# avlmaps/AVLMaps

Measured on AMD Instinct MI355X. Metric: voxel_query_similarities_per_sec, higher is better.
Workload: dtype f32

## Files before the change

avlmaps_amd/_lib.py:

```python
from __future__ import annotations

import ctypes as C
import os
import sys
import threading
from pathlib import Path

_PKG = Path(__file__).resolve().parent
LIB_PATH = Path(os.environ.get("AVLMAPS_HIP_LIB") or _PKG / "lib" / "libavlmaps_hip.so")

AVL_OK = 0
SIM_AUTO, SIM_EXACT, SIM_SPLIT_F16, SIM_EXACT_VALU, SIM_PREPARED, SIM_PREPARED24 = 0, 1, 2, 3, 4, 5


class AvlError(RuntimeError):
    pass


_lib = None

_vp, _i32, _i64, _f64, _sz = C.c_void_p, C.c_int32, C.c_int64, C.c_double, C.c_size_t
_SIGS = {
    "avl_last_error": (C.c_char_p, []),
    "avl_version": (C.c_int, []),
# ... 68 lines not shown
    "avl_builder_destroy": (C.c_int, [_vp]),
    "avl_builder_reset": (C.c_int, [_vp, _vp]),
    "avl_builder_enable_replay_log": (C.c_int, [_vp, _i64]),
    "avl_builder_integrate_frame": (C.c_int, [_vp, _vp, C.c_int, C.c_int, _vp, _vp, _vp, _vp, C.c_int, _vp, C.c_int,
                                              C.c_int, _vp, _i64, _f64, _f64, _f64, _vp]),
    "avl_builder_integrate_batch": (C.c_int, [_vp, C.c_int, _vp, C.c_int, C.c_int, _vp, _vp, _vp, _vp, C.c_int, _vp, C.c_int, C.c_int,
                                              _vp, _i64, _f64, _f64, _f64, _vp]),
    "avl_builder_integrate_frames": (C.c_int, [_vp, C.c_int, _vp, C.c_int, C.c_int, _vp, _vp, _vp, _vp, C.c_int, _vp, C.c_int, C.c_int,
                                               _vp, _i64, _f64, _f64, _f64, _vp]),
    "avl_builder_integrate_frame_global": (C.c_int, [_vp, _vp, C.c_int, _f64, C.c_int, C.c_int, _vp, _vp, _vp, _vp, C.c_int, _vp,
                                                     C.c_int, C.c_int, _vp, _i64, _f64, _f64, _f64, _vp, _vp]),
    "avl_points_bbox": (C.c_int, [_vp, C.c_int, _f64, C.c_int, C.c_int, _vp, _vp, _vp, C.c_int, _f64, _f64, _vp, _vp]),
    "avl_builder_import_map": (C.c_int, [_vp, _i64, _vp, _vp, _vp, _vp, _vp]),
    "avl_builder_num_voxels": (C.c_int, [_vp, C.POINTER(_i64), _vp]),
    "avl_builder_num_points": (C.c_int, [_vp, C.POINTER(_i64), _vp]),
    "avl_builder_num_groups": (C.c_int, [_vp, C.POINTER(_i64), _vp]),
    "avl_builder_finalize": (C.c_int, [_vp, _i64, _vp, _vp, _vp, _vp, _vp, _vp]),
    "avl_builder_finalize_ex": (C.c_int, [_vp, _i64, _vp, _vp, _vp, _vp, _vp, _vp, C.c_int, _vp]),
    "avl_builder_export_raw": (C.c_int, [_vp, _i64, _vp, _vp, _vp, _vp, _vp, _vp, _vp]),
    "avl_finalize_raw": (C.c_int, [_i64, C.c_int, C.c_int, C.c_int, _vp, _vp, _vp, _vp, _vp, _vp, _vp, _vp, _vp, _vp, _vp]),
    "avl_builder_set_max_capacity": (C.c_int, [_vp, _i64]),
    "avl_builder_capacity": (C.c_int, [_vp, C.POINTER(_i64)]),
    "avl_builder_set_deferred_fuse": (C.c_int, [_vp, C.c_int, _vp]),
    "avl_builder_flush": (C.c_int, [_vp, _vp]),
    "avl_builder_release_scratch": (C.c_int, [_vp, _i64, _vp]),
    "avl_builder_scatter_merge": (C.c_int, [_vp, _i64, _vp, _vp, _vp, _i64, _vp]),
    "avl_finalize_merged": (C.c_int, [_i64, _i64, C.c_int, C.c_int, C.c_int, _vp, _vp, _i64, _vp, _vp, _vp, _vp, _vp, _vp]),
    "avl_builder_replay_chain": (C.c_int, [_vp, _i64, _vp, C.c_uint64, _vp, _vp]),
    "avl_builder_drop_replay_cache": (C.c_int, [_vp, _vp]),
    "avl_builder_replay_prepare": (C.c_int, [_vp, _i64, _vp]),
    "avl_replay_state_apply": (C.c_int, [_i64, _vp, _vp, _vp, _vp]),
    "avl_rows_add_f64": (C.c_int, [_i64, C.c_int, _vp, _i64, _i64, _vp, _i64, _vp, _i64, _vp]),
    "avl_rows_add_f64_async": (C.c_int, [_i64, C.c_int, _vp, _i64, _i64, _vp, _i64, _vp, _i64, _vp, _vp]),
    "avl_builder_export_rows_f32": (C.c_int, [_vp, _i64, _vp, _vp, _i64, _vp]),
    "avl_builder_export_rows_f64": (C.c_int, [_vp, _i64, _vp, _vp, _vp, _i64, _vp]),
    "avl_finalize_side": (C.c_int, [_i64, _i64, C.c_int, C.c_int, _vp, _vp, _vp, _vp, _vp, _vp, _vp]),
    "avl_pool_label_2d": (C.c_int, [_vp, _vp, _i64, C.c_int, _vp, _vp]),
    "avl_rgb_topdown": (C.c_int, [_vp, _vp, _i64, C.c_int, _vp, _vp]),
    "avl_obstacle_map": (C.c_int, [_vp, C.c_int, C.c_int, C.c_int, C.c_int, C.c_int, _vp, _vp]),
    "avl_obstacle_scatter": (C.c_int, [_vp, _vp, _i64, _vp, C.c_int, C.c_int, C.c_int, C.c_int, C.c_int, _vp, _vp, _vp]),
    "avl_heatmap_from_mask": (C.c_int, [_vp, _vp, _i64, _f64, _f64, _vp, _vp]),
    "avl_heat_plan_create": (C.c_int, [C.POINTER(_vp), _vp, _i64, _vp]),
    "avl_heat_plan_destroy": (C.c_int, [_vp]),
    "avl_heatmap_from_mask_planned": (C.c_int, [_vp, _vp, _f64, _f64, _vp, _vp]),
    "avl_lseg_merge_windows": (C.c_int, [_vp, C.c_int, C.c_int, C.c_int, C.c_int, _vp, C.c_int, C.c_int, _vp, _vp]),
    "avl_field_area": (C.c_int, [_vp, _vp, _i64, C.c_int, _f64, _vp, _vp, _vp]),
# ... 72 lines not shown
```

avlmaps_amd/csrc/avl_builder.hip:

```cpp
#include <algorithm>
#include <climits>
#include <cstring>
#include <vector>

#include <rocprim/device/device_radix_sort.hpp>
#include <rocprim/device/device_select.hpp>
#include <rocprim/iterator/counting_iterator.hpp>

#include "avl_common.h"

namespace avl {

#ifdef AVL_PROBE_CHAIN
__device__ unsigned long long* g_probe = nullptr;
constexpr int kProbeK12Row0 = 16384;
#define AVL_STAMP(var)                                                                                             \
    unsigned long long var;                                                                                        \
    asm volatile("s_waitcnt vmcnt(0) lgkmcnt(0)\n\ts_memrealtime %0\n\ts_waitcnt lgkmcnt(0)" : "=s"(var)::"memory")
#define AVL_STAMP_DECL(var) unsigned long long var = 0
#define AVL_RESTAMP(var) asm volatile("s_waitcnt vmcnt(0) lgkmcnt(0)\n\ts_memrealtime %0\n\ts_waitcnt lgkmcnt(0)" : "=s"(var)::"memory")
#else
#define AVL_STAMP(var)
#define AVL_STAMP_DECL(var)
#define AVL_RESTAMP(var)
// ... 75 lines not shown
    const auto p = __builtin_amdgcn_kernarg_segment_ptr();
    int t0, t1, t2, t3;
    if constexpr (LINES == 4)
        asm volatile("s_load_dword %0, %4, 0x0\n s_load_dword %1, %4, 0x40\n s_load_dword %2, %4, 0x80\n s_load_dword %3, %4, 0xc0\n"
                     "s_waitcnt lgkmcnt(0)" : "=&s"(t0), "=&s"(t1), "=&s"(t2), "=&s"(t3) : "s"(p));
    if constexpr (LINES == 8)
        asm volatile("s_load_dword %0, %4, 0x0\n s_load_dword %1, %4, 0x40\n s_load_dword %2, %4, 0x80\n s_load_dword %3, %4, 0xc0\n"
                     "s_load_dword %0, %4, 0x100\n s_load_dword %1, %4, 0x140\n s_load_dword %2, %4, 0x180\n s_load_dword %3, %4, 0x1c0\n"
                     "s_waitcnt lgkmcnt(0)" : "=&s"(t0), "=&s"(t1), "=&s"(t2), "=&s"(t3) : "s"(p));
    if constexpr (LINES == 12)
        asm volatile("s_load_dword %0, %4, 0x0\n s_load_dword %1, %4, 0x40\n s_load_dword %2, %4, 0x80\n s_load_dword %3, %4, 0xc0\n"
                     "s_load_dword %0, %4, 0x100\n s_load_dword %1, %4, 0x140\n s_load_dword %2, %4, 0x180\n s_load_dword %3, %4, 0x1c0\n"
                     "s_load_dword %0, %4, 0x200\n s_load_dword %1, %4, 0x240\n s_load_dword %2, %4, 0x280\n s_load_dword %3, %4, 0x2c0\n"
                     "s_waitcnt lgkmcnt(0)" : "=&s"(t0), "=&s"(t1), "=&s"(t2), "=&s"(t3) : "s"(p));
    if constexpr (LINES == 16)
        asm volatile("s_load_dword %0, %4, 0x0\n s_load_dword %1, %4, 0x40\n s_load_dword %2, %4, 0x80\n s_load_dword %3, %4, 0xc0\n"
                     "s_load_dword %0, %4, 0x100\n s_load_dword %1, %4, 0x140\n s_load_dword %2, %4, 0x180\n s_load_dword %3, %4, 0x1c0\n"
                     "s_load_dword %0, %4, 0x200\n s_load_dword %1, %4, 0x240\n s_load_dword %2, %4, 0x280\n s_load_dword %3, %4, 0x2c0\n"
                     "s_load_dword %0, %4, 0x300\n s_load_dword %1, %4, 0x340\n s_load_dword %2, %4, 0x380\n s_load_dword %3, %4, 0x3c0\n"
                     "s_waitcnt lgkmcnt(0)" : "=&s"(t0), "=&s"(t1), "=&s"(t2), "=&s"(t3) : "s"(p));
    (void)t0; (void)t1; (void)t2; (void)t3;
    __builtin_amdgcn_sched_barrier(0);
#endif
}

__device__ __forceinline__ int py_int(double v) {
    return (int)fmin(fmax(v, -2.0e9), 2.0e9);
}

__device__ __forceinline__ double gemv3(const double* a, double x0, double x1, double x2) {
    return fma(a[2], x2, fma(a[0], x0, a[1] * x1));
}

struct SampleRec {
    double alpha;
    int32_t cell, fpix;
    uint32_t rgbv;
    int32_t slot;
};

template <int THREADS, int MODE = 0>
__device__ __forceinline__ SampleRec bp_voxelize_body(int blk, const FrameParams& fp, const float* depth,
                                                      const int32_t* __restrict__ sample_idx, const uint8_t* rgb,
                                                      int32_t* __restrict__ cell_slot, int32_t* __restrict__ slot_cell, const Recs& recs,
                                                      unsigned long long* __restrict__ counters, int* __restrict__ err_flags,
                                                      PreRec* __restrict__ pre_out = nullptr) {
// ... 271 lines not shown
    warm_kernel_arguments<12>();
    const SampleRec r = bp_voxelize_body<256>(blockIdx.x, fp, depth, sample_idx, rgb, cell_slot, slot_cell, recs, counters, err_flags);
    link_body<true, 256>(blockIdx.x, fp.P, cell_slot, head, recs, counters, log, log_base, frame_key, fp.batch, fp.P_frame, r, err_flags, ol);
}

__global__ __launch_bounds__(256) void voxelize_link_next_kernel(FrameParams fp, const float* depth, const int32_t* __restrict__ sample_idx,
                                                                 const uint8_t* rgb, int32_t* __restrict__ cell_slot,
                                                                 int32_t* __restrict__ slot_cell, Recs recs, int32_t* __restrict__ head,
                                                                 unsigned long long* __restrict__ counters, int* __restrict__ err_flags,
                                                                 ReplayLog log, long long log_base, unsigned long long frame_key,
                                                                 FrameParams fpn, PreGather next, int gb) {
    if ((int)blockIdx.x < gb) {
        bp_voxelize_body<256, 2>((int)blockIdx.x, fpn, next.depth, next.samples, next.rgb, cell_slot, slot_cell, recs, counters, err_flags, next.out);
        return;
    }
    const int blk = (int)blockIdx.x - gb;
    warm_kernel_arguments<12>();
    SampleRec r;
    if (fp.pre) r = bp_voxelize_body<256, 1>(blk, fp, depth, sample_idx, rgb, cell_slot, slot_cell, recs, counters, err_flags);
    else r = bp_voxelize_body<256, 0>(blk, fp, depth, sample_idx, rgb, cell_slot, slot_cell, recs, counters, err_flags);
    link_body<false, 256>(blk, fp.P, cell_slot, head, recs, counters, log, log_base, frame_key, nullptr, fp.P_frame, r, err_flags);
}

template <int CH, bool FULL>
__device__ __forceinline__ void fuse_group_impl(int s0, int32_t slot, double alpha0, int32_t fpix0, uint32_t rgb0, int P, int D_rt, unsigned long long frame_key, const BatchEntry* __restrict__ batch,
                                                int P_frame, const Recs& recs, int32_t* __restrict__ head, const float* __restrict__ feat,
                                                double* __restrict__ sum_feat, double* __restrict__ sum_w4,
                                                float* __restrict__ first_feat, double* __restrict__ first_alpha,
                                                unsigned long long* __restrict__ slot_key, uint8_t* __restrict__ dirty) {
    const int D = FULL ? 256 * CH : D_rt;
    const int lane = threadIdx.x & 63;
    AVL_STAMP(pt0);
    AVL_STAMP(pt1);
    const bool is_new = slot_key[slot] == kNoKey;
    const int h0 = head[slot];
    double* sf = sum_feat + (size_t)slot * D;
    AVL_STAMP(pt2);
#ifdef AVL_PROBE_CHAIN
    int probe_n = 1;
    unsigned long long pt3 = 0, pt4 = 0;
#endif

    double acc[CH][4], old[CH][4];
    float f1[CH][4];
#pragma unroll
    for (int c = 0; c < CH; ++c)
#pragma unroll
        for (int e = 0; e < 4; ++e) { acc[c][e] = 0.0; f1[c][e] = 0.f; old[c][e] = 0.0; }
    double w4 = 0.0, a1 = 0.0, w4_old = 0.0;
    int min_s = INT_MAX;
    if (!is_new) {
#pragma unroll
        for (int c = 0; c < CH; ++c) {
            const int d = c * 256 + lane * 4;
            if (FULL || (d + 3 < D && (D & 1) == 0)) {
                const double2 q0 = *reinterpret_cast<const double2*>(sf + d), q1 = *reinterpret_cast<const double2*>(sf + d + 2);
                old[c][0] = q0.x; old[c][1] = q0.y; old[c][2] = q1.x; old[c][3] = q1.y;
            } else {
#pragma unroll
                for (int e = 0; e < 4; ++e)
                    if (d + e < D) old[c][e] = sf[d + e];
            }
        }
    }
    if (lane < 4) w4_old = is_new ? 0.0 : sum_w4[(size_t)slot * 4 + lane];

    auto row_of = [&](int cur, int32_t fpix) { return (batch ? batch[cur / P_frame].feat : feat) + (size_t)fpix * D; };
    auto load_row = [&](float (&v)[CH][4], const float* f) {
#pragma unroll
        for (int c = 0; c < CH; ++c) {
            const int d = c * 256 + lane * 4;
            if (FULL || (d + 3 < D && (D & 3) == 0)) {
                const float4 q = *reinterpret_cast<const float4*>(f + d);
// ... 23 lines not shown
        }
        if (lane < 4) w4 += lane == 0 ? alpha : alpha * (double)((rgbv >> (8 * (lane - 1))) & 0xffu);
    };
    const float* feat0 = row_of(s0, fpix0);
#ifdef AVL_ABL_K3_SINGLE
    if (true) {
#else
    if (h0 == s0) {
#endif
        float v[CH][4];
        load_row(v, feat0);
        add(s0, alpha0, rgb0, v);
#ifdef AVL_PROBE_CHAIN
        { AVL_STAMP(ptx); pt3 = pt4 = ptx; }
#endif
    } else {
        int my = lane == 0 ? s0 : INT_MAX;
        int n = 1, cur = h0;
        while (cur != s0 && n < 64 && (unsigned)cur < (unsigned)P) {
            if (lane == n) my = cur;
            ++n;
            cur = recs.next[cur];
        }
#ifdef AVL_PROBE_CHAIN
        { AVL_STAMP(ptx); pt3 = ptx; probe_n = n; }
#endif
        double a_l = 0.0;
        int32_t fp_l = 0;
        uint32_t rgb_l = 0;
        if (lane < n) {
            a_l = recs.alpha[my];
            fp_l = recs.fpix[my];
            rgb_l = recs.rgb[my];
        }
#ifdef AVL_PROBE_CHAIN
        { AVL_STAMP(ptx); pt4 = ptx; }
#endif
        int rank = 0;
        for (int j = 0; j < n; ++j) rank += __builtin_amdgcn_readlane(my, j) < my ? 1 : 0;
        const int a_lo = __double2loint(a_l), a_hi = __double2hiint(a_l);
#ifndef AVL_K3_MR
#define AVL_K3_MR 2
#endif
        constexpr int MR = CH <= 4 ? AVL_K3_MR : 1;
        for (int k0 = 0; k0 < n; k0 += MR) {
            float v[MR][CH][4];
            int cj[MR], lj[MR];
#pragma unroll
            for (int j = 0; j < MR; ++j) {
                const unsigned long long m = __ballot(lane < n && rank == k0 + j);
                lj[j] = m ? __builtin_amdgcn_readfirstlane(__ffsll((long long)m) - 1) : 0;
                cj[j] = m ? __builtin_amdgcn_readlane(my, lj[j]) : -1;
                load_row(v[j], cj[j] >= 0 ? row_of(cj[j], __builtin_amdgcn_readlane(fp_l, lj[j])) : feat0);
            }
#pragma unroll
            for (int j = 0; j < MR; ++j) {
                if (cj[j] >= 0) {
                    const double al = __hiloint2double(__builtin_amdgcn_readlane(a_hi, lj[j]), __builtin_amdgcn_readlane(a_lo, lj[j]));
                    add(cj[j], al, (uint32_t)__builtin_amdgcn_readlane((int)rgb_l, lj[j]), v[j]);
                }
            }
        }
        for (int steps = 0; cur != s0 && (unsigned)cur < (unsigned)P && steps < P; ++steps) {
            const int nxt = recs.next[cur];
            float v[CH][4];
            load_row(v, row_of(cur, recs.fpix[cur]));
            add(cur, recs.alpha[cur], recs.rgb[cur], v);
            cur = nxt;
        }
    }

    AVL_STAMP(pt5);
    float* ff = first_feat + (size_t)slot * D;
#pragma unroll
    for (int c = 0; c < CH; ++c) {
        const int d = c * 256 + lane * 4;
        double r[4];
#pragma unroll
        for (int e = 0; e < 4; ++e) r[e] = is_new ? acc[c][e] : old[c][e] + acc[c][e];
        if constexpr (FULL) {
            *reinterpret_cast<double2*>(sf + d) = double2{r[0], r[1]};
            *reinterpret_cast<double2*>(sf + d + 2) = double2{r[2], r[3]};
            if (is_new) *reinterpret_cast<float4*>(ff + d) = float4{f1[c][0], f1[c][1], f1[c][2], f1[c][3]};
        } else {
#pragma unroll
            for (int e = 0; e < 4; ++e)
                if (d + e < D) {
                    sf[d + e] = r[e];
                    if (is_new) ff[d + e] = f1[c][e];
                }
        }
    }
    if (lane < 4) sum_w4[(size_t)slot * 4 + lane] = w4_old + w4;
    if (is_new) {
        if (lane == 0) {
            first_alpha[slot] = a1;
            slot_key[slot] = batch ? (batch[min_s / P_frame].frame_key | (unsigned)(min_s % P_frame)) : (frame_key | (unsigned)min_s);
        }
    }
    if (lane == 0) {
        head[slot] = -1;
        dirty[slot] = 1;
    }
#ifdef AVL_PROBE_CHAIN
    {
        AVL_STAMP(pt6);
        if (g_probe && lane == 0 && P < kProbeK12Row0) {
            unsigned long long* q = g_probe + (size_t)s0 * 8;
            q[0] = pt0; q[1] = pt1; q[2] = pt2; q[3] = pt3; q[4] = pt4; q[5] = pt5; q[6] = pt6;
            q[7] = (unsigned long long)probe_n | (is_new ? 1ull << 32 : 0ull);
        }
    }
#endif
}

template <int CH, bool COMPACT = false>
__device__ __forceinline__ void fuse_body(int blk, int P, int D, unsigned long long frame_key, const BatchEntry* __restrict__ batch,
                                          int P_frame, const Recs& recs, int32_t* __restrict__ head, const float* __restrict__ feat,
                                          double* __restrict__ sum_feat, double* __restrict__ sum_w4,
                                          float* __restrict__ first_feat, double* __restrict__ first_alpha,
                                          unsigned long long* __restrict__ slot_key, uint8_t* __restrict__ dirty,
                                          const OwnerList& ol = OwnerList{}) {
    auto group = [&](int s0, int32_t slot, double alpha0, int32_t fpix0, uint32_t rgb0) {
        if (D == 256 * CH)
            fuse_group_impl<CH, true>(s0, slot, alpha0, fpix0, rgb0, P, D, frame_key, batch, P_frame, recs, head, feat, sum_feat, sum_w4, first_feat,
                                      first_alpha, slot_key, dirty);
        else
            fuse_group_impl<CH, false>(s0, slot, alpha0, fpix0, rgb0, P, D, frame_key, batch, P_frame, recs, head, feat, sum_feat, sum_w4, first_feat,
                                       first_alpha, slot_key, dirty);
    };
    if constexpr (!COMPACT) {
        const int s0 = __builtin_amdgcn_readfirstlane((int)((blk * AVL_K3_THREADS + threadIdx.x) >> 6));
        if (s0 >= P) return;
        const uint8_t own = recs.owner[s0];
        const int32_t slot = recs.slot[s0];
        const double alpha0 = recs.alpha[s0];
        const int32_t fpix0 = recs.fpix[s0];
        const uint32_t rgb0 = recs.rgb[s0];
        if (!own) return;
        group(s0, slot, alpha0, fpix0, rgb0);
        return;
    } else {
    const int nb = (P + 255) / 256;
    const int nblk = nb * (kFuseWaves / 4);
    const int t = (int)(threadIdx.x >> 6) * nblk + blk;
    const int b = __builtin_amdgcn_readfirstlane(t / kFuseWaves);
    if (b >= nb) return;
    const int n_own = __builtin_amdgcn_readfirstlane(ol.ocnt[b]);
    for (int k = t % kFuseWaves; k < n_own; k += kFuseWaves) {
        const int oi = __builtin_amdgcn_readfirstlane(b * 256 + k);
        const double a0 = ol.o_alpha[oi];
        group(__builtin_amdgcn_readfirstlane(ol.o_s[oi]), __builtin_amdgcn_readfirstlane(ol.o_slot[oi]),
              __hiloint2double(__builtin_amdgcn_readfirstlane(__double2hiint(a0)), __builtin_amdgcn_readfirstlane(__double2loint(a0))),
              __builtin_amdgcn_readfirstlane(ol.o_fpix[oi]), (uint32_t)__builtin_amdgcn_readfirstlane((int)ol.o_rgb[oi]));
    }
    }
}

#ifndef AVL_K3_WPE
#define AVL_K3_WPE 0
#endif
#if AVL_K3_WPE
#define AVL_K3_OCC(CH) __attribute__((amdgpu_waves_per_eu((CH) <= 2 ? AVL_K3_WPE : 1)))
#else
#define AVL_K3_OCC(CH)
#endif

template <int CH, bool COMPACT>
__global__ __launch_bounds__(COMPACT ? 256 : AVL_K3_THREADS) AVL_K3_OCC(CH) void fuse_kernel(int P, int D, unsigned long long frame_key, const BatchEntry* __restrict__ batch,
                                                   int P_frame, Recs recs, int32_t* __restrict__ head, const float* __restrict__ feat,
                                                   double* __restrict__ sum_feat, double* __restrict__ sum_w4,
                                                   float* __restrict__ first_feat, double* __restrict__ first_alpha,
                                                   unsigned long long* __restrict__ slot_key, uint8_t* __restrict__ dirty, OwnerList ol) {
    fuse_body<CH, COMPACT>(blockIdx.x, P, D, frame_key, batch, P_frame, recs, head, feat, sum_feat, sum_w4, first_feat, first_alpha, slot_key, dirty, ol);
}

struct FusePrev {
    int P;
    unsigned long long frame_key;
    Recs recs;
    int32_t* head;
    const float* feat;
};

template <int CH>
__global__ __launch_bounds__(AVL_K3_THREADS) AVL_K3_OCC(CH) void pipe_kernel(FrameParams fp, int pb, const float* depth, const int32_t* __restrict__ sample_idx,
                                                   const uint8_t* rgb, int32_t* __restrict__ cell_slot, int32_t* __restrict__ slot_cell,
                                                   Recs recs, int32_t* __restrict__ head, unsigned long long* __restrict__ counters,
                                                   int* __restrict__ err_flags, ReplayLog log, long long log_base,
                                                   unsigned long long frame_key, FusePrev prev, int D, double* __restrict__ sum_feat,
                                                   double* __restrict__ sum_w4, float* __restrict__ first_feat,
                                                   double* __restrict__ first_alpha, unsigned long long* __restrict__ slot_key,
                                                   uint8_t* __restrict__ dirty, FrameParams fpn, PreGather next, int gb) {
    if ((int)blockIdx.x < gb) {
        bp_voxelize_body<AVL_K3_THREADS, 2>((int)blockIdx.x, fpn, next.depth, next.samples, next.rgb, cell_slot, slot_cell, recs, counters, err_flags,
                                            next.out);
        return;
// ... 7 lines not shown
        link_body<false, AVL_K3_THREADS>(blk, fp.P, cell_slot, head, recs, counters, log, log_base, frame_key, nullptr, fp.P_frame, r, err_flags);
    } else {
        fuse_body<CH>(blk - pb, prev.P, D, prev.frame_key, nullptr, prev.P, prev.recs, prev.head, prev.feat, sum_feat, sum_w4,
                      first_feat, first_alpha, slot_key, dirty);
    }
}

constexpr int kGenTile = 8;
__global__ __launch_bounds__(256) void fuse_generic_kernel(int P, int D, unsigned long long frame_key,
                                                           const BatchEntry* __restrict__ batch, int P_frame, Recs recs,
                                                           int32_t* __restrict__ head, const float* __restrict__ feat,
                                                           double* __restrict__ sum_feat, double* __restrict__ sum_w4,
                                                           float* __restrict__ first_feat, double* __restrict__ first_alpha,
                                                           unsigned long long* __restrict__ slot_key, uint8_t* __restrict__ dirty) {
    __shared__ int ord_s[4][64];
    const int lane = threadIdx.x & 63;
    int* ord = ord_s[(threadIdx.x >> 6) & 3];
    const int s0 = (blockIdx.x * blockDim.x + threadIdx.x) >> 6;
    if (s0 >= P) return;
    if (!recs.owner[s0]) return;
    const int32_t slot = recs.slot[s0];
    const bool is_new = slot_key[slot] == kNoKey;
    const int h0 = head[slot];
    auto wave_max = [&](int v) {
#pragma unroll
        for (int o = 32; o >= 1; o >>= 1) v = max(v, __shfl_xor(v, o));
        return v;
    };
    int n_total = 0, min_s = INT_MAX, held = INT_MAX;
    for (int cur = h0; cur >= 0 && (unsigned)cur < (unsigned)P && n_total < P; cur = recs.next[cur]) {
        if (n_total < 64 && lane == n_total) held = cur;
        min_s = min(min_s, cur);
        ++n_total;
    }
    if (n_total == 0) return;
    const double a1 = recs.alpha[min_s];
    const float* row1 = (batch ? batch[min_s / P_frame].feat : feat) + (size_t)recs.fpix[min_s] * D;
    double* sf = sum_feat + (size_t)slot * D;
    float* ff = first_feat + (size_t)slot * D;
    if (is_new)
        for (int d = lane; d < D; d += 64) ff[d] = row1[d];
    double w4 = 0.0;
    int prev = -1;
    bool first_round = true;
    for (int done = 0; done < n_total;) {
        int m;
        if (n_total <= 64) {
            m = n_total;
        } else {
            held = INT_MAX;
            int cnt = 0, curmax = -1, steps = 0;
            for (int cur = h0; cur >= 0 && (unsigned)cur < (unsigned)P && steps < P; cur = recs.next[cur], ++steps) {
                if (cur <= prev) continue;
                if (cnt < 64) {
                    if (lane == cnt) held = cur;
                    if (++cnt == 64) curmax = wave_max(held);
                } else if (cur < curmax) {
                    const unsigned long long at = __ballot(held == curmax);
                    if (lane == __ffsll((long long)at) - 1) held = cur;
                    curmax = wave_max(held);
                }
            }
            m = cnt;
            if (m == 0) break;
        }
        int rank = 0;
        for (int j = 0; j < m; ++j) rank += __builtin_amdgcn_readlane(held, j) < held ? 1 : 0;
        if (lane < m) ord[rank] = held;
        __builtin_amdgcn_wave_barrier();
        prev = ord[m - 1];
        for (int k = 0; k < m; ++k) {
            const int cur = ord[k];
            const double alpha = recs.alpha[cur];
            const uint32_t rgbv = recs.rgb[cur];
            if (lane < 4) w4 += lane == 0 ? alpha : alpha * (double)((rgbv >> (8 * (lane - 1))) & 0xffu);
        }
        for (int d0 = 0; d0 < D; d0 += 64 * kGenTile) {
            double acc[kGenTile];
#pragma unroll
            for (int t = 0; t < kGenTile; ++t) acc[t] = 0.0;
            for (int k = 0; k < m; ++k) {
                const int cur = ord[k];
                if (is_new && cur == min_s) continue;
                const double alpha = recs.alpha[cur];
                const float* row = (batch ? batch[cur / P_frame].feat : feat) + (size_t)recs.fpix[cur] * D;
#pragma unroll
                for (int t = 0; t < kGenTile; ++t) {
                    const int d = d0 + t * 64 + lane;
                    if (d < D) acc[t] += alpha * (double)row[d];
                }
            }
#pragma unroll
            for (int t = 0; t < kGenTile; ++t) {
                const int d = d0 + t * 64 + lane;
                if (d < D) sf[d] = (is_new && first_round) ? acc[t] : sf[d] + acc[t];
            }
        }
        __builtin_amdgcn_wave_barrier();
        done += m;
        first_round = false;
    }
    if (lane < 4) {
        double* w = sum_w4 + (size_t)slot * 4 + lane;
        *w = is_new ? w4 : *w + w4;
    }
    if (lane == 0) {
        if (is_new) {
            first_alpha[slot] = a1;
            slot_key[slot] = batch ? (batch[min_s / P_frame].frame_key | (unsigned)(min_s % P_frame)) : (frame_key | (unsigned)min_s);
        }
        head[slot] = -1;
        dirty[slot] = 1;
    }
}

__global__ __launch_bounds__(256) void finalize_kernel(int64_t n, int D, int gs, int vh, int64_t row0, const int32_t* __restrict__ perm,
                                                       const int32_t* __restrict__ cell, const double* __restrict__ sum_feat,
                                                       int64_t ld_sf, const double* __restrict__ sum_w4, int64_t ld_w4,
                                                       const float* __restrict__ first_feat, const double* __restrict__ first_alpha,
                                                       float* __restrict__ grid_feat, int32_t* __restrict__ grid_pos,
                                                       float* __restrict__ weight, uint8_t* __restrict__ grid_rgb,
                                                       int32_t* __restrict__ occupied) {
    const int lane = threadIdx.x & 63;
    const int64_t wave0 = ((int64_t)blockIdx.x * blockDim.x + threadIdx.x) >> 6;
    const int64_t nwaves = ((int64_t)gridDim.x * blockDim.x) >> 6;
    for (int64_t r = wave0; r < n; r += nwaves) {
        const int64_t sl = perm ? perm[r] : r;
        const double w = sum_w4[sl * ld_w4];
// ... 359 lines not shown
struct LogSegments;
struct avl_builder {
    int n0, gs, vh, D;
    double cs;
    int64_t capacity;
    size_t ncell;
    int32_t* cell_slot = nullptr;
    int32_t* slot_cell = nullptr;
    unsigned long long* slot_key = nullptr;
    double* sum_feat = nullptr;
    double* sum_w4 = nullptr;
    float* first_feat = nullptr;
    double* first_alpha = nullptr;
    int32_t* head = nullptr;
    int32_t* head_alt = nullptr;
    uint8_t* dirty = nullptr;
    unsigned long long* counters = nullptr;
    int* err_flags = nullptr;
    char* recs_mem = nullptr;
    OwnerList owners{};
    Recs recs{}, recs_alt{};
    int recs_cap = 0;
    int deferred = 0;
    struct Pending {
        int P = 0;
        unsigned long long frame_key = 0;
        const float* feat = nullptr;
    } pend;
    unsigned long long key_bias = 0;
    ReplayLog log{};
    long long log_cap = 0, log_used = 0;
    char* rs_mem = nullptr;
    size_t rs_bytes = 0;
    size_t rs_tmp_bytes = 0;
    BatchEntry* d_table = nullptr;
    int table_cap = 0;
    int64_t vox_bound = 0;
    int64_t max_capacity = 0;
    LogSegments* ls_cache = nullptr;
    long long ls_log_used = -1;
    int64_t ls_n = -1;

    PreRec* pre_buf[2] = {nullptr, nullptr};
    struct PreHeld {
        FrameParams fp{};
        const int32_t* samples = nullptr;
// ... 248 lines not shown
        if (block2) (void)hipFreeAsync(block2, st);
        if (block1) (void)hipFreeAsync(block1, st);
        block1 = block2 = nullptr;
    }
};

static void drop_log_segments(avl_builder* b, hipStream_t st) {
    if (!b->ls_cache) return;
    b->ls_cache->release(st);
    delete b->ls_cache;
    b->ls_cache = nullptr;
    b->ls_log_used = -1;
    b->ls_n = -1;
}

static int launch_fuse(avl_builder* b, int P, unsigned long long frame_key, const BatchEntry* batch, int P_frame, const Recs& recs,
                       int32_t* head, const float* d_feat, hipStream_t st, bool owners_compacted) {
    const bool compact = owners_compacted && b->D <= 1536 && P >= kAggregateSamples;
    constexpr int kWaves = AVL_K3_THREADS / 64;
    const unsigned wb = compact ? (unsigned)((P + 255) / 256) * (kFuseWaves / 4) : (unsigned)((P + kWaves - 1) / kWaves);
#define AVL_FUSE_LAUNCH(CH)                                                                                                              \
    do {                                                                                                                                 \
        if (compact)                                                                                                                     \
            hipLaunchKernelGGL((fuse_kernel<CH, true>), dim3(wb), dim3(256), 0, st, P, b->D, frame_key, batch, P_frame, recs, head, d_feat,  \
                               b->sum_feat, b->sum_w4, b->first_feat, b->first_alpha, b->slot_key, b->dirty, b->owners);                 \
        else                                                                                                                             \
            hipLaunchKernelGGL((fuse_kernel<CH, false>), dim3(wb), dim3(AVL_K3_THREADS), 0, st, P, b->D, frame_key, batch, P_frame, recs, head, d_feat, \
                               b->sum_feat, b->sum_w4, b->first_feat, b->first_alpha, b->slot_key, b->dirty, OwnerList{});               \
    } while (0)
    if (b->D <= 256) AVL_FUSE_LAUNCH(1);
    else if (b->D <= 512) AVL_FUSE_LAUNCH(2);
    else if (b->D == 768) AVL_FUSE_LAUNCH(3);
    else if (b->D <= 1024) AVL_FUSE_LAUNCH(4);
    else if (b->D <= 1536) AVL_FUSE_LAUNCH(6);
    else
        hipLaunchKernelGGL(fuse_generic_kernel, dim3(wb), dim3(256), 0, st, P, b->D, frame_key, batch, P_frame, recs, head, d_feat,
                           b->sum_feat, b->sum_w4, b->first_feat, b->first_alpha, b->slot_key, b->dirty);
#undef AVL_FUSE_LAUNCH
    AVL_HIP_CHECK(hipGetLastError());
    return AVL_OK;
}

static int flush_pending(avl_builder* b, hipStream_t st) {
    if (b->pend.P == 0) return AVL_OK;
    const int P = b->pend.P;
    b->pend.P = 0;
    return launch_fuse(b, P, b->pend.frame_key, nullptr, P, b->recs_alt, b->head_alt, b->pend.feat, st, false);
}

template <int CH>
static void launch_pipe(avl_builder* b, const FrameParams& fp, unsigned pb, const void* d_depth, const int32_t* d_sample_idx,
// ... 330 lines not shown
}

int avl_builder_integrate_frame_global(avl_builder* b, const void* d_depth, int depth_is_u16, double depth_div, int H, int W,
                                       const double* h_calib, const double* h_calib_inv, const double* h_transform,
                                       const int32_t* d_sample_idx, int P, const float* d_feat, int Hf, int Wf,
                                       const uint8_t* d_rgb, int64_t frame_idx, double min_depth, double max_depth,
                                       double sigma_sq, const double* h_pcd_min, void* stream) {
    AVL_REQUIRE(h_pcd_min, "avl_builder_integrate_frame_global: pcd_min is required");
    AVL_REQUIRE(!depth_is_u16 || depth_div > 0, "avl_builder_integrate_frame_global: depth_div must be positive");
    return integrate_impl(b, d_depth, depth_is_u16 ? 1 : 0, depth_div, H, W, h_calib, h_calib_inv, h_transform, d_sample_idx, P, d_feat,
                          Hf, Wf, d_rgb, frame_idx, min_depth, max_depth, sigma_sq, h_pcd_min, stream);
}

int avl_builder_integrate_batch(avl_builder* b, int B, const float* const* h_depth_ptrs, int H, int W, const double* h_calib,
                                const double* h_calib_inv, const double* h_pc_transforms, const int32_t* const* h_sample_ptrs, int P,
                                const float* const* h_feat_ptrs, int Hf, int Wf, const uint8_t* const* h_rgb_ptrs, int64_t frame_idx0,
                                double min_depth, double max_depth, double sigma_sq, void* stream) {
    AVL_REQUIRE(B > 0, "avl_builder_integrate_batch: B must be positive");
    return integrate_impl(b, nullptr, 0, 1.0, H, W, h_calib, h_calib_inv, h_pc_transforms, nullptr, P, nullptr, Hf, Wf, nullptr, frame_idx0,
                          min_depth, max_depth, sigma_sq, nullptr, stream, B, reinterpret_cast<const void* const*>(h_depth_ptrs),
                          h_sample_ptrs, h_feat_ptrs, h_rgb_ptrs);
}

int avl_builder_integrate_frames(avl_builder* b, int n_frames, const float* const* h_depth_ptrs, int H, int W, const double* h_calib,
                                 const double* h_calib_inv, const double* h_pc_transforms, const int32_t* const* h_sample_ptrs, int P,
                                 const float* const* h_feat_ptrs, int Hf, int Wf, const uint8_t* const* h_rgb_ptrs, int64_t frame_idx0,
                                 double min_depth, double max_depth, double sigma_sq, void* stream) {
    AVL_REQUIRE(n_frames > 0, "avl_builder_integrate_frames: n_frames must be positive");
    AVL_REQUIRE(h_depth_ptrs && h_sample_ptrs && h_feat_ptrs && h_rgb_ptrs && h_pc_transforms, "avl_builder_integrate_frames: null pointer table");
    AVL_REQUIRE(b, "avl_builder_integrate_frames: null handle");
    for (int i = 0; i < n_frames; ++i) {
        b->pre_next = {};
        if (i + 1 < n_frames && h_sample_ptrs[i + 1] && h_depth_ptrs[i + 1] && h_rgb_ptrs[i + 1])
            b->pre_next = {h_sample_ptrs[i + 1], h_depth_ptrs[i + 1], h_rgb_ptrs[i + 1], h_pc_transforms + 16 * (i + 1)};
        const int rc = integrate_impl(b, h_depth_ptrs[i], 0, 1.0, H, W, h_calib, h_calib_inv, h_pc_transforms + 16 * i, h_sample_ptrs[i], P,
                                      h_feat_ptrs[i], Hf, Wf, h_rgb_ptrs[i], frame_idx0 + i, min_depth, max_depth, sigma_sq, nullptr, stream);
        b->pre_next = {};
        if (rc != AVL_OK) return rc;
    }
    return AVL_OK;
}

int avl_builder_num_voxels(avl_builder* b, int64_t* h_n, void* stream) {
    AVL_REQUIRE(b && h_n, "avl_builder_num_voxels: null argument");
    int rc = flush_pending(b, as_stream(stream));
    if (rc != AVL_OK) return rc;
    rc = builder_check_flags(b, as_stream(stream));
    if (rc != AVL_OK) return rc;
    rc = read_counter(b, 0, h_n, as_stream(stream));
    if (rc == AVL_OK && *h_n > b->capacity) *h_n = b->capacity;
    return rc;
}

int avl_builder_num_points(avl_builder* b, int64_t* h_n, void* stream) {
    AVL_REQUIRE(b && h_n, "avl_builder_num_points: null argument");
    if (int rc = flush_pending(b, as_stream(stream)); rc != AVL_OK) return rc;
    return read_counter(b, 1, h_n, as_stream(stream));
}

int avl_builder_num_groups(avl_builder* b, int64_t* h_n, void* stream) {
    AVL_REQUIRE(b && h_n, "avl_builder_num_groups: null argument");
// ... 527 lines not shown
```

avlmaps_amd/ops.py:

```python
from __future__ import annotations

import ctypes as C

import numpy as np

from . import _lib
from .device import DeviceArray, as_device, _is_torch

PRECISION = {"auto": _lib.SIM_AUTO, "exact": _lib.SIM_EXACT, "split_f16": _lib.SIM_SPLIT_F16, "exact_valu": _lib.SIM_EXACT_VALU,
             "prepared": _lib.SIM_PREPARED}


def query_col_support(queries):
    q = np.asarray(queries)
    nz = q != 0
    any_nz = nz.any(axis=1)
    begin = np.where(any_nz, nz.argmax(axis=1), 0).astype(np.int32)
    end = np.where(any_nz, q.shape[1] - nz[:, ::-1].argmax(axis=1), 0).astype(np.int32)
    return begin, end


def sim_scores(feat, queries, want_scores=True, want_argmax=True, want_best=False, precision="auto", stream=None,
               out_scores=None, out_argmax=None, out_best=None, col_support="auto"):
    lib = _lib.load()
    _lib.require_gpu()
# ... 205 lines not shown


class VoxelAccumulator:

    def __init__(self, gs, cs, vh, D, capacity=None, n_rows=None, max_capacity=None, deferred_fuse=False):
        lib = _lib.load()
        _lib.require_gpu()
        self.gs, self.cs, self.vh, self.D = int(gs), float(cs), int(vh), int(D)
        self.n_rows = int(n_rows) if n_rows else self.gs
        ncell = self.n_rows * self.gs * self.vh
        cap0 = int(capacity) if capacity else min(self.n_rows * self.gs, ncell)
        h = C.c_void_p()
        _lib.check(lib.avl_builder_create_grid(C.byref(h), self.n_rows, self.gs, self.vh, self.cs, self.D, cap0),
                   "avl_builder_create_grid")
        self._h = h
        self._has_log = False
        self._max_frame, self._imported = 0, False
        if max_capacity is None:
            max_capacity = min(ncell, (1 << 31) - 1)
        if max_capacity and max_capacity > cap0:
            _lib.check(lib.avl_builder_set_max_capacity(h, int(max_capacity)), "avl_builder_set_max_capacity")
        if deferred_fuse:
            self.set_deferred_fuse(True)

    def _retain(self, keeps, stream):
        self._keep_prev, self._keep = getattr(self, "_keep", None), keeps
        if not any(isinstance(k, DeviceArray) for k in keeps):
            return
        lib = _lib.load()
        q = self.__dict__.setdefault("_keep_events", [])
        free = self.__dict__.setdefault("_free_events", [])
        if free:
            ev = free.pop()
        else:
            ev = C.c_void_p()
            _lib.check(lib.avl_event_create(C.byref(ev)), "avl_event_create")
        _lib.check(lib.avl_event_record(ev, stream), "avl_event_record")
        q.append((ev, keeps))
        while len(q) > 4:
            old_ev, _old = q.pop(0)
            _lib.check(lib.avl_event_sync(q[0][0] if getattr(self, "_deferred", False) else old_ev), "avl_event_sync")
            free.append(old_ev)

    def _calib_pair(self, calib, calib_inv):
        K = np.ascontiguousarray(np.asarray(calib, dtype=np.float64).reshape(3, 3))
        if calib_inv is not None:
            return K, np.ascontiguousarray(np.asarray(calib_inv, dtype=np.float64).reshape(3, 3))
        key = K.tobytes()
        c = getattr(self, "_kinv_cache", None)
        if c is None or c[0] != key:
            c = self._kinv_cache = (key, np.ascontiguousarray(np.linalg.inv(K)))
        return K, c[1]

    def key_bits(self) -> int:
        return 63 if self._imported else 32 + max(1, int(self._max_frame).bit_length())

    def set_deferred_fuse(self, on, stream=None):
        _lib.check(_lib.load().avl_builder_set_deferred_fuse(self._h, int(bool(on)), stream), "avl_builder_set_deferred_fuse")
        self._deferred = bool(on)
        return self

    def flush(self, stream=None):
        _lib.check(_lib.load().avl_builder_flush(self._h, stream), "avl_builder_flush")
        return self

    def release_scratch(self, keep_bytes=0, stream=None):
        _lib.check(_lib.load().avl_builder_release_scratch(self._h, int(keep_bytes), stream), "avl_builder_release_scratch")
        return self

    @property
    def capacity(self):
        c = C.c_int64()
        _lib.check(_lib.load().avl_builder_capacity(self._h, C.byref(c)), "avl_builder_capacity")
        return c.value

    def has_replay_log(self):
        return self._has_log

    def drop_replay_cache(self):
        from .device import torch_stream_ptr
        _lib.check(_lib.load().avl_builder_drop_replay_cache(self._h, torch_stream_ptr()), "avl_builder_drop_replay_cache")

# ... 577 lines not shown
```

include/avlmaps_hip.h:

```cpp
#ifndef AVLMAPS_HIP_H
#define AVLMAPS_HIP_H

#include <stddef.h>
#include <stdint.h>

#ifdef __cplusplus
extern "C" {
#endif

#define AVL_API __attribute__((visibility("default")))

enum {
    AVL_OK = 0,
    AVL_ERR_INVALID = 1,
    AVL_ERR_HIP = 2,
    AVL_ERR_CAPACITY = 3,
    AVL_ERR_NO_DEVICE = 4,
    AVL_ERR_STATE = 5
};

AVL_API const char* avl_last_error(void);
AVL_API int avl_version(void);
AVL_API int avl_device_count(int* h_count);
AVL_API int avl_set_device(int device);
// ... 78 lines not shown
AVL_API int avl_builder_create_grid(avl_builder** h_out, int n0, int n1, int n2, double cs, int D, int64_t capacity);
AVL_API int avl_builder_destroy(avl_builder* b);
AVL_API int avl_builder_reset(avl_builder* b, void* stream);
AVL_API int avl_builder_set_max_capacity(avl_builder* b, int64_t max_capacity);
AVL_API int avl_builder_capacity(avl_builder* b, int64_t* h_capacity);
AVL_API int avl_builder_set_deferred_fuse(avl_builder* b, int on, void* stream);
AVL_API int avl_builder_flush(avl_builder* b, void* stream);
AVL_API int avl_builder_release_scratch(avl_builder* b, int64_t keep_bytes, void* stream);

AVL_API int avl_builder_enable_replay_log(avl_builder* b, int64_t max_samples);

AVL_API int avl_builder_integrate_frame(avl_builder* b, const float* d_depth, int H, int W, const double* h_calib,
                                        const double* h_calib_inv, const double* h_pc_transform,
                                        const int32_t* d_sample_idx, int P, const float* d_feat, int Hf, int Wf,
                                        const uint8_t* d_rgb, int64_t frame_idx, double min_depth,
                                        double max_depth, double sigma_sq, void* stream);

AVL_API int avl_builder_integrate_batch(avl_builder* b, int B, const float* const* h_depth_ptrs, int H, int W,
                                        const double* h_calib, const double* h_calib_inv, const double* h_pc_transforms,
                                        const int32_t* const* h_sample_ptrs, int P, const float* const* h_feat_ptrs, int Hf,
                                        int Wf, const uint8_t* const* h_rgb_ptrs, int64_t frame_idx0, double min_depth,
                                        double max_depth, double sigma_sq, void* stream);

AVL_API int avl_builder_integrate_frames(avl_builder* b, int n_frames, const float* const* h_depth_ptrs, int H, int W,
                                        const double* h_calib, const double* h_calib_inv, const double* h_pc_transforms,
                                        const int32_t* const* h_sample_ptrs, int P, const float* const* h_feat_ptrs, int Hf,
                                        int Wf, const uint8_t* const* h_rgb_ptrs, int64_t frame_idx0, double min_depth,
                                        double max_depth, double sigma_sq, void* stream);

AVL_API int avl_builder_integrate_frame_global(avl_builder* b, const void* d_depth, int depth_is_u16, double depth_div, int H,
                                               int W, const double* h_calib, const double* h_calib_inv,
                                               const double* h_transform, const int32_t* d_sample_idx, int P,
                                               const float* d_feat, int Hf, int Wf, const uint8_t* d_rgb, int64_t frame_idx,
                                               double min_depth, double max_depth, double sigma_sq, const double* h_pcd_min,
                                               void* stream);

AVL_API int avl_points_bbox(const void* d_depth, int depth_is_u16, double depth_div, int H, int W, const double* h_calib_inv,
                            const double* h_transform, const int32_t* d_sample_idx, int P, double min_depth, double max_depth,
                            double* h_minmax, void* stream);

AVL_API int avl_builder_import_map(avl_builder* b, int64_t n, const float* d_grid_feat, const int32_t* d_grid_pos,
                                   const float* d_weight, const uint8_t* d_grid_rgb, void* stream);

AVL_API int avl_builder_num_voxels(avl_builder* b, int64_t* h_n, void* stream);
AVL_API int avl_builder_num_points(avl_builder* b, int64_t* h_n, void* stream);
AVL_API int avl_builder_num_groups(avl_builder* b, int64_t* h_n, void* stream);
// ... 119 lines not shown
```

Before: 180.0 billion.

## Batch consecutive frames into grouped integrate calls with per-frame ordered fusion

integrate_frames now processes groups of up to 64 frames (configurable) through the batched integrate path, where previously each frame had its own call. The fuse kernels gain a MULTI mode. It walks a voxel's sample chain in index-ordered rounds of 64 and folds accumulators at frame boundaries, so the per-frame summation order matches sequential integration. This is meant to cut per-frame launch and host overhead during map building. In exchange, fusion gets more complex, with a round-based chain scan that can repeat traversal of long chains.

After: 180.2 billion (median of 6 runs). About the same (+0.1%).

```diff
diff --git a/avlmaps_amd/_lib.py b/avlmaps_amd/_lib.py
--- a/avlmaps_amd/_lib.py
+++ b/avlmaps_amd/_lib.py
@@ -114,6 +114,7 @@
     "avl_builder_set_max_capacity": (C.c_int, [_vp, _i64]),
     "avl_builder_capacity": (C.c_int, [_vp, C.POINTER(_i64)]),
     "avl_builder_set_deferred_fuse": (C.c_int, [_vp, C.c_int, _vp]),
+    "avl_builder_set_frame_group": (C.c_int, [_vp, C.c_int]),
     "avl_builder_flush": (C.c_int, [_vp, _vp]),
     "avl_builder_release_scratch": (C.c_int, [_vp, _i64, _vp]),
     "avl_builder_scatter_merge": (C.c_int, [_vp, _i64, _vp, _vp, _vp, _i64, _vp]),
diff --git a/avlmaps_amd/csrc/avl_builder.hip b/avlmaps_amd/csrc/avl_builder.hip
--- a/avlmaps_amd/csrc/avl_builder.hip
+++ b/avlmaps_amd/csrc/avl_builder.hip
@@ -121,6 +121,12 @@
     (void)t0; (void)t1; (void)t2; (void)t3;
     __builtin_amdgcn_sched_barrier(0);
 #endif
+}
+
+__device__ __forceinline__ int wave_max_i32(int v) {
+#pragma unroll
+    for (int o = 32; o >= 1; o >>= 1) v = max(v, __shfl_xor(v, o));
+    return __builtin_amdgcn_readfirstlane(v);
 }
 
 __device__ __forceinline__ int py_int(double v) {
@@ -438,7 +444,7 @@
     link_body<false, 256>(blk, fp.P, cell_slot, head, recs, counters, log, log_base, frame_key, nullptr, fp.P_frame, r, err_flags);
 }
 
-template <int CH, bool FULL>
+template <int CH, bool FULL, bool MULTI>
 __device__ __forceinline__ void fuse_group_impl(int s0, int32_t slot, double alpha0, int32_t fpix0, uint32_t rgb0, int P, int D_rt, unsigned long long frame_key, const BatchEntry* __restrict__ batch,
                                                 int P_frame, const Recs& recs, int32_t* __restrict__ head, const float* __restrict__ feat,
                                                 double* __restrict__ sum_feat, double* __restrict__ sum_w4,
@@ -465,6 +471,7 @@
         for (int e = 0; e < 4; ++e) { acc[c][e] = 0.0; f1[c][e] = 0.f; old[c][e] = 0.0; }
     double w4 = 0.0, a1 = 0.0, w4_old = 0.0;
     int min_s = INT_MAX;
+    int fr_end = 0;
     if (!is_new) {
 #pragma unroll
         for (int c = 0; c < CH; ++c) {
@@ -534,51 +541,88 @@
             ++n;
             cur = recs.next[cur];
         }
+        const bool rounds = cur != s0 && (unsigned)cur < (unsigned)P;
 #ifdef AVL_PROBE_CHAIN
         { AVL_STAMP(ptx); pt3 = ptx; probe_n = n; }
 #endif
-        double a_l = 0.0;
-        int32_t fp_l = 0;
-        uint32_t rgb_l = 0;
-        if (lane < n) {
-            a_l = recs.alpha[my];
-            fp_l = recs.fpix[my];
-            rgb_l = recs.rgb[my];
-        }
+        int prev = -1;
+        for (;;) {
+            if (rounds) {
+                my = INT_MAX;
+                n = 0;
+                int curmax = -1;
+                for (int c = h0, steps = 0; (unsigned)c < (unsigned)P && steps < P; c = recs.next[c], ++steps) {
+                    if (c <= prev) continue;
+                    if (n < 64) {
+                        if (lane == n) my = c;
+                        if (++n == 64) curmax = wave_max_i32(my);
+                    } else if (c < curmax) {
+                        const unsigned long long at = __ballot(my == curmax);
+                        if (lane == __ffsll((long long)at) - 1) my = c;
+                        curmax = wave_max_i32(my);
+                    }
+                }
+            }
+            double a_l = 0.0;
+            int32_t fp_l = 0;
+            uint32_t rgb_l = 0;
+            if (lane < n) {
+                a_l = recs.alpha[my];
+                fp_l = recs.fpix[my];
+                rgb_l = recs.rgb[my];
+            }
 #ifdef AVL_PROBE_CHAIN
-        { AVL_STAMP(ptx); pt4 = ptx; }
+            { AVL_STAMP(ptx); pt4 = ptx; }
 #endif
-        int rank = 0;
-        for (int j = 0; j < n; ++j) rank += __builtin_amdgcn_readlane(my, j) < my ? 1 : 0;
-        const int a_lo = __double2loint(a_l), a_hi = __double2hiint(a_l);
+            int rank = 0;
+            for (int j = 0; j < n; ++j) rank += __builtin_amdgcn_readlane(my, j) < my ? 1 : 0;
+            const int a_lo = __double2loint(a_l), a_hi = __double2hiint(a_l);
 #ifndef AVL_K3_MR
 #define AVL_K3_MR 2
 #endif
-        constexpr int MR = CH <= 4 ? AVL_K3_MR : 1;
-        for (int k0 = 0; k0 < n; k0 += MR) {
-            float v[MR][CH][4];
-            int cj[MR], lj[MR];
+            constexpr int MR = CH <= 4 ? AVL_K3_MR : 1;
+            for (int k0 = 0; k0 < n;) {
+                float v[MR][CH][4];
+                int cj[MR], lj[MR];
 #pragma unroll
-            for (int j = 0; j < MR; ++j) {
-                const unsigned long long m = __ballot(lane < n && rank == k0 + j);
-                lj[j] = m ? __builtin_amdgcn_readfirstlane(__ffsll((long long)m) - 1) : 0;
-                cj[j] = m ? __builtin_amdgcn_readlane(my, lj[j]) : -1;
-                load_row(v[j], cj[j] >= 0 ? row_of(cj[j], __builtin_amdgcn_readlane(fp_l, lj[j])) : feat0);
-            }
+                for (int j = 0; j < MR; ++j) {
+                    const unsigned long long m = __ballot(lane < n && rank == k0 + j);
+                    lj[j] = m ? __builtin_amdgcn_readfirstlane(__ffsll((long long)m) - 1) : 0;
+                    cj[j] = m ? __builtin_amdgcn_readlane(my, lj[j]) : -1;
+                }
+                if (MULTI && cj[0] >= fr_end) {
+                    if (fr_end > 0) {
 #pragma unroll
-            for (int j = 0; j < MR; ++j) {
-                if (cj[j] >= 0) {
-                    const double al = __hiloint2double(__builtin_amdgcn_readlane(a_hi, lj[j]), __builtin_amdgcn_readlane(a_lo, lj[j]));
-                    add(cj[j], al, (uint32_t)__builtin_amdgcn_readlane((int)rgb_l, lj[j]), v[j]);
+                        for (int c = 0; c < CH; ++c)
+#pragma unroll
+                            for (int e = 0; e < 4; ++e) {
+                                old[c][e] += acc[c][e];
+                                acc[c][e] = 0.0;
+                            }
+                        w4_old += w4;
+                        w4 = 0.0;
+                    }
+                    fr_end = (cj[0] / P_frame + 1) * P_frame;
+                }
+                int taken = 1;
+#pragma unroll
+                for (int j = 1; j < MR; ++j) {
+                    if (MULTI && cj[j] >= fr_end) cj[j] = -1;
+                    taken += cj[j] >= 0 ? 1 : 0;
+                }
+                k0 += taken;
+#pragma unroll
+                for (int j = 0; j < MR; ++j) load_row(v[j], cj[j] >= 0 ? row_of(cj[j], __builtin_amdgcn_readlane(fp_l, lj[j])) : feat0);
+#pragma unroll
+                for (int j = 0; j < MR; ++j) {
+                    if (cj[j] >= 0) {
+                        const double al = __hiloint2double(__builtin_amdgcn_readlane(a_hi, lj[j]), __builtin_amdgcn_readlane(a_lo, lj[j]));
+                        add(cj[j], al, (uint32_t)__builtin_amdgcn_readlane((int)rgb_l, lj[j]), v[j]);
+                    }
                 }
             }
-        }
-        for (int steps = 0; cur != s0 && (unsigned)cur < (unsigned)P && steps < P; ++steps) {
-            const int nxt = recs.next[cur];
-            float v[CH][4];
-            load_row(v, row_of(cur, recs.fpix[cur]));
-            add(cur, recs.alpha[cur], recs.rgb[cur], v);
-            cur = nxt;
+            if (!rounds || n < 64) break;
+            prev = wave_max_i32(my);
         }
     }
 
@@ -589,7 +633,7 @@
         const int d = c * 256 + lane * 4;
         double r[4];
 #pragma unroll
-        for (int e = 0; e < 4; ++e) r[e] = is_new ? acc[c][e] : old[c][e] + acc[c][e];
+        for (int e = 0; e < 4; ++e) r[e] = old[c][e] + acc[c][e];
         if constexpr (FULL) {
             *reinterpret_cast<double2*>(sf + d) = double2{r[0], r[1]};
             *reinterpret_cast<double2*>(sf + d + 2) = double2{r[2], r[3]};
@@ -626,7 +670,7 @@
 #endif
 }
 
-template <int CH, bool COMPACT = false>
+template <int CH, bool COMPACT = false, bool MULTI = COMPACT>
 __device__ __forceinline__ void fuse_body(int blk, int P, int D, unsigned long long frame_key, const BatchEntry* __restrict__ batch,
                                           int P_frame, const Recs& recs, int32_t* __restrict__ head, const float* __restrict__ feat,
                                           double* __restrict__ sum_feat, double* __restrict__ sum_w4,
@@ -635,10 +679,10 @@
                                           const OwnerList& ol = OwnerList{}) {
     auto group = [&](int s0, int32_t slot, double alpha0, int32_t fpix0, uint32_t rgb0) {
         if (D == 256 * CH)
-            fuse_group_impl<CH, true>(s0, slot, alpha0, fpix0, rgb0, P, D, frame_key, batch, P_frame, recs, head, feat, sum_feat, sum_w4, first_feat,
+            fuse_group_impl<CH, true, MULTI>(s0, slot, alpha0, fpix0, rgb0, P, D, frame_key, batch, P_frame, recs, head, feat, sum_feat, sum_w4, first_feat,
                                       first_alpha, slot_key, dirty);
         else
-            fuse_group_impl<CH, false>(s0, slot, alpha0, fpix0, rgb0, P, D, frame_key, batch, P_frame, recs, head, feat, sum_feat, sum_w4, first_feat,
+            fuse_group_impl<CH, false, MULTI>(s0, slot, alpha0, fpix0, rgb0, P, D, frame_key, batch, P_frame, recs, head, feat, sum_feat, sum_w4, first_feat,
                                        first_alpha, slot_key, dirty);
     };
     if constexpr (!COMPACT) {
@@ -678,13 +722,13 @@
 #define AVL_K3_OCC(CH)
 #endif
 
-template <int CH, bool COMPACT>
+template <int CH, bool COMPACT, bool MULTI>
 __global__ __launch_bounds__(COMPACT ? 256 : AVL_K3_THREADS) AVL_K3_OCC(CH) void fuse_kernel(int P, int D, unsigned long long frame_key, const BatchEntry* __restrict__ batch,
                                                    int P_frame, Recs recs, int32_t* __restrict__ head, const float* __restrict__ feat,
                                                    double* __restrict__ sum_feat, double* __restrict__ sum_w4,
                                                    float* __restrict__ first_feat, double* __restrict__ first_alpha,
                                                    unsigned long long* __restrict__ slot_key, uint8_t* __restrict__ dirty, OwnerList ol) {
-    fuse_body<CH, COMPACT>(blockIdx.x, P, D, frame_key, batch, P_frame, recs, head, feat, sum_feat, sum_w4, first_feat, first_alpha, slot_key, dirty, ol);
+    fuse_body<CH, COMPACT, MULTI>(blockIdx.x, P, D, frame_key, batch, P_frame, recs, head, feat, sum_feat, sum_w4, first_feat, first_alpha, slot_key, dirty, ol);
 }
 
 struct FusePrev {
@@ -738,11 +782,7 @@
     const int32_t slot = recs.slot[s0];
     const bool is_new = slot_key[slot] == kNoKey;
     const int h0 = head[slot];
-    auto wave_max = [&](int v) {
-#pragma unroll
-        for (int o = 32; o >= 1; o >>= 1) v = max(v, __shfl_xor(v, o));
-        return v;
-    };
+    auto frame_of = [&](int cur) { return batch ? cur / P_frame : 0; };
     int n_total = 0, min_s = INT_MAX, held = INT_MAX;
     for (int cur = h0; cur >= 0 && (unsigned)cur < (unsigned)P && n_total < P; cur = recs.next[cur]) {
         if (n_total < 64 && lane == n_total) held = cur;
@@ -756,35 +796,45 @@
     float* ff = first_feat + (size_t)slot * D;
     if (is_new)
         for (int d = lane; d < D; d += 64) ff[d] = row1[d];
-    double w4 = 0.0;
-    int prev = -1;
+    double w4 = 0.0, w4_run = 0.0;
+    if (lane < 4 && !is_new) w4_run = sum_w4[(size_t)slot * 4 + lane];
+    bool have_w = !is_new;
+    int prev = -1, fr = -1;
     bool first_round = true;
     for (int done = 0; done < n_total;) {
-        int m;
-        if (n_total <= 64) {
-            m = n_total;
-        } else {
+        if (n_total > 64) {
             held = INT_MAX;
             int cnt = 0, curmax = -1, steps = 0;
             for (int cur = h0; cur >= 0 && (unsigned)cur < (unsigned)P && steps < P; cur = recs.next[cur], ++steps) {
                 if (cur <= prev) continue;
                 if (cnt < 64) {
                     if (lane == cnt) held = cur;
-                    if (++cnt == 64) curmax = wave_max(held);
+                    if (++cnt == 64) curmax = wave_max_i32(held);
                 } else if (cur < curmax) {
                     const unsigned long long at = __ballot(held == curmax);
                     if (lane == __ffsll((long long)at) - 1) held = cur;
-                    curmax = wave_max(held);
+                    curmax = wave_max_i32(held);
                 }
             }
-            m = cnt;
-            if (m == 0) break;
-        }
+            if (cnt == 0) break;
+        }
+        const int cand = held > prev && held != INT_MAX ? held : INT_MAX;
         int rank = 0;
-        for (int j = 0; j < m; ++j) rank += __builtin_amdgcn_readlane(held, j) < held ? 1 : 0;
-        if (lane < m) ord[rank] = held;
+        for (int j = 0; j < min(n_total, 64); ++j) rank += __builtin_amdgcn_readlane(cand, j) < cand ? 1 : 0;
+        if (cand != INT_MAX) ord[rank] = cand;
         __builtin_amdgcn_wave_barrier();
+        const int f = frame_of(ord[0]);
+        const int m = __popcll(__ballot(cand != INT_MAX && frame_of(cand) == f));
+        if (m == 0) break;
         prev = ord[m - 1];
+        if (f != fr) {
+            if (fr >= 0) {
+                w4_run = have_w ? w4_run + w4 : w4;
+                have_w = true;
+                w4 = 0.0;
+            }
+            fr = f;
+        }
         for (int k = 0; k < m; ++k) {
             const int cur = ord[k];
             const double alpha = recs.alpha[cur];
@@ -816,10 +866,7 @@
         done += m;
         first_round = false;
     }
-    if (lane < 4) {
-        double* w = sum_w4 + (size_t)slot * 4 + lane;
-        *w = is_new ? w4 : *w + w4;
-    }
+    if (lane < 4) sum_w4[(size_t)slot * 4 + lane] = have_w ? w4_run + w4 : w4;
     if (lane == 0) {
         if (is_new) {
             first_alpha[slot] = a1;
@@ -1225,6 +1272,7 @@
     Recs recs{}, recs_alt{};
     int recs_cap = 0;
     int deferred = 0;
+    int frame_group = 64;
     struct Pending {
         int P = 0;
         unsigned long long frame_key = 0;
@@ -1519,11 +1567,14 @@
 #define AVL_FUSE_LAUNCH(CH)                                                                                                              \
     do {                                                                                                                                 \
         if (compact)                                                                                                                     \
-            hipLaunchKernelGGL((fuse_kernel<CH, true>), dim3(wb), dim3(256), 0, st, P, b->D, frame_key, batch, P_frame, recs, head, d_feat,  \
+            hipLaunchKernelGGL((fuse_kernel<CH, true, true>), dim3(wb), dim3(256), 0, st, P, b->D, frame_key, batch, P_frame, recs, head, d_feat,  \
                                b->sum_feat, b->sum_w4, b->first_feat, b->first_alpha, b->slot_key, b->dirty, b->owners);                 \
+        else if (batch)                                                                                                                  \
+            hipLaunchKernelGGL((fuse_kernel<CH, false, true>), dim3(wb), dim3(AVL_K3_THREADS), 0, st, P, b->D, frame_key, batch, P_frame, recs, head, \
+                               d_feat, b->sum_feat, b->sum_w4, b->first_feat, b->first_alpha, b->slot_key, b->dirty, OwnerList{});       \
         else                                                                                                                             \
-            hipLaunchKernelGGL((fuse_kernel<CH, false>), dim3(wb), dim3(AVL_K3_THREADS), 0, st, P, b->D, frame_key, batch, P_frame, recs, head, d_feat, \
-                               b->sum_feat, b->sum_w4, b->first_feat, b->first_alpha, b->slot_key, b->dirty, OwnerList{});               \
+            hipLaunchKernelGGL((fuse_kernel<CH, false, false>), dim3(wb), dim3(AVL_K3_THREADS), 0, st, P, b->D, frame_key, batch, P_frame, recs, head, \
+                               d_feat, b->sum_feat, b->sum_w4, b->first_feat, b->first_alpha, b->slot_key, b->dirty, OwnerList{});       \
     } while (0)
     if (b->D <= 256) AVL_FUSE_LAUNCH(1);
     else if (b->D <= 512) AVL_FUSE_LAUNCH(2);
@@ -1900,6 +1951,13 @@
                           h_sample_ptrs, h_feat_ptrs, h_rgb_ptrs);
 }
 
+int avl_builder_set_frame_group(avl_builder* b, int frames) {
+    AVL_REQUIRE(b, "avl_builder_set_frame_group: null handle");
+    AVL_REQUIRE(frames >= 1 && frames <= 4096, "avl_builder_set_frame_group: frames must be in [1, 4096]");
+    b->frame_group = frames;
+    return AVL_OK;
+}
+
 int avl_builder_integrate_frames(avl_builder* b, int n_frames, const float* const* h_depth_ptrs, int H, int W, const double* h_calib,
                                  const double* h_calib_inv, const double* h_pc_transforms, const int32_t* const* h_sample_ptrs, int P,
                                  const float* const* h_feat_ptrs, int Hf, int Wf, const uint8_t* const* h_rgb_ptrs, int64_t frame_idx0,
@@ -1907,14 +1965,24 @@
     AVL_REQUIRE(n_frames > 0, "avl_builder_integrate_frames: n_frames must be positive");
     AVL_REQUIRE(h_depth_ptrs && h_sample_ptrs && h_feat_ptrs && h_rgb_ptrs && h_pc_transforms, "avl_builder_integrate_frames: null pointer table");
     AVL_REQUIRE(b, "avl_builder_integrate_frames: null handle");
-    for (int i = 0; i < n_frames; ++i) {
-        b->pre_next = {};
-        if (i + 1 < n_frames && h_sample_ptrs[i + 1] && h_depth_ptrs[i + 1] && h_rgb_ptrs[i + 1])
-            b->pre_next = {h_sample_ptrs[i + 1], h_depth_ptrs[i + 1], h_rgb_ptrs[i + 1], h_pc_transforms + 16 * (i + 1)};
-        const int rc = integrate_impl(b, h_depth_ptrs[i], 0, 1.0, H, W, h_calib, h_calib_inv, h_pc_transforms + 16 * i, h_sample_ptrs[i], P,
-                                      h_feat_ptrs[i], Hf, Wf, h_rgb_ptrs[i], frame_idx0 + i, min_depth, max_depth, sigma_sq, nullptr, stream);
-        b->pre_next = {};
+    const int G = b->frame_group;
+    for (int i = 0; i < n_frames;) {
+        const int g = std::min(G, n_frames - i);
+        int rc;
+        if (g > 1) {
+            rc = integrate_impl(b, nullptr, 0, 1.0, H, W, h_calib, h_calib_inv, h_pc_transforms + 16 * i, nullptr, P, nullptr, Hf, Wf, nullptr,
+                                frame_idx0 + i, min_depth, max_depth, sigma_sq, nullptr, stream, g,
+                                reinterpret_cast<const void* const*>(h_depth_ptrs + i), h_sample_ptrs + i, h_feat_ptrs + i, h_rgb_ptrs + i);
+        } else {
+            b->pre_next = {};
+            if (i + 1 < n_frames && h_sample_ptrs[i + 1] && h_depth_ptrs[i + 1] && h_rgb_ptrs[i + 1])
+                b->pre_next = {h_sample_ptrs[i + 1], h_depth_ptrs[i + 1], h_rgb_ptrs[i + 1], h_pc_transforms + 16 * (i + 1)};
+            rc = integrate_impl(b, h_depth_ptrs[i], 0, 1.0, H, W, h_calib, h_calib_inv, h_pc_transforms + 16 * i, h_sample_ptrs[i], P,
+                                h_feat_ptrs[i], Hf, Wf, h_rgb_ptrs[i], frame_idx0 + i, min_depth, max_depth, sigma_sq, nullptr, stream);
+            b->pre_next = {};
+        }
         if (rc != AVL_OK) return rc;
+        i += g;
     }
     return AVL_OK;
 }
diff --git a/avlmaps_amd/ops.py b/avlmaps_amd/ops.py
--- a/avlmaps_amd/ops.py
+++ b/avlmaps_amd/ops.py
@@ -1,6 +1,7 @@
 from __future__ import annotations
 
 import ctypes as C
+import os
 
 import numpy as np
 
@@ -252,6 +253,9 @@
             _lib.check(lib.avl_builder_set_max_capacity(h, int(max_capacity)), "avl_builder_set_max_capacity")
         if deferred_fuse:
             self.set_deferred_fuse(True)
+        fg = os.environ.get("AVLMAPS_FRAME_GROUP")
+        if fg:
+            self.set_frame_group(int(fg))
 
     def _retain(self, keeps, stream):
         self._keep_prev, self._keep = getattr(self, "_keep", None), keeps
@@ -288,6 +292,10 @@
     def set_deferred_fuse(self, on, stream=None):
         _lib.check(_lib.load().avl_builder_set_deferred_fuse(self._h, int(bool(on)), stream), "avl_builder_set_deferred_fuse")
         self._deferred = bool(on)
+        return self
+
+    def set_frame_group(self, frames):
+        _lib.check(_lib.load().avl_builder_set_frame_group(self._h, int(frames)), "avl_builder_set_frame_group")
         return self
 
     def flush(self, stream=None):
diff --git a/include/avlmaps_hip.h b/include/avlmaps_hip.h
--- a/include/avlmaps_hip.h
+++ b/include/avlmaps_hip.h
@@ -124,6 +124,7 @@
                                         int Wf, const uint8_t* const* h_rgb_ptrs, int64_t frame_idx0, double min_depth,
                                         double max_depth, double sigma_sq, void* stream);
 
+AVL_API int avl_builder_set_frame_group(avl_builder* b, int frames);
 AVL_API int avl_builder_integrate_frames(avl_builder* b, int n_frames, const float* const* h_depth_ptrs, int H, int W,
                                         const double* h_calib, const double* h_calib_inv, const double* h_pc_transforms,
                                         const int32_t* const* h_sample_ptrs, int P, const float* const* h_feat_ptrs, int Hf,
```
